# tyui592/Real_Time_Helmet_Detection

Measured on AMD Instinct MI355X. Metric: train imgs/sec, higher is better.
Workload: dtype bf16; 1 GPU; model=hourglass-1-ch128, global_batch=16, imsize=512, parallelism=dp1, engine=hip, fp8=False, hipgraph=True

## Files before the change

### real_time_helmet_detection_amd/ops/csrc/bindings.cpp

```cpp
#include <torch/extension.h>

namespace rthd {
torch::Tensor add_act_fwd(torch::Tensor a, torch::Tensor b, int64_t act);
torch::Tensor add_act_bwd(torch::Tensor dy, torch::Tensor y, int64_t act);

std::vector<torch::Tensor> pool2x2_fwd(torch::Tensor x, bool is_max,
                                       bool need_arg);
torch::Tensor pool2x2_bwd(torch::Tensor dy, torch::Tensor arg, bool is_max,
                          int64_t H, int64_t W);
std::vector<torch::Tensor> maxpool_same_fwd(torch::Tensor x, int64_t k,
                                            bool need_arg);
torch::Tensor maxpool_same_bwd(torch::Tensor dy, torch::Tensor arg,
                               int64_t k);

torch::Tensor upsample2x_add_fwd(torch::Tensor x,
                                 c10::optional<torch::Tensor> skip);
torch::Tensor upsample2x_bwd(torch::Tensor dy);

std::vector<torch::Tensor> centernet_loss_fwd(
    torch::Tensor phm, torch::Tensor poff, torch::Tensor psize,
    torch::Tensor ghm, torch::Tensor goff, torch::Tensor gsize,
    torch::Tensor mask, double alpha, double beta);
std::vector<torch::Tensor> centernet_loss_bwd(
    torch::Tensor phm, torch::Tensor poff, torch::Tensor psize,
    torch::Tensor ghm, torch::Tensor goff, torch::Tensor gsize,
    torch::Tensor mask, torch::Tensor sums, torch::Tensor gout,
    double alpha, double beta);
std::vector<torch::Tensor> centernet_loss_fused_fwd(
    torch::Tensor out, torch::Tensor ghm, torch::Tensor goff,
    torch::Tensor gsize, torch::Tensor mask, double alpha, double beta,
    bool sig_os);
torch::Tensor centernet_loss_fused_bwd(
    torch::Tensor out, torch::Tensor ghm, torch::Tensor goff,
    torch::Tensor gsize, torch::Tensor mask, torch::Tensor sums,
    torch::Tensor glosses, double alpha, double beta, bool sig_os);

std::vector<torch::Tensor> decode_fwd(torch::Tensor hm, torch::Tensor off,
                                      torch::Tensor wh, int64_t scale_factor,
                                      int64_t topk, int64_t pool_size,
                                      bool normalized);
torch::Tensor nms_fwd(torch::Tensor boxes, torch::Tensor scores,
                      double iou_threshold);
std::vector<torch::Tensor> nms_batched(torch::Tensor boxes,
                                       torch::Tensor scores,
                                       double iou_threshold,
                                       double conf_th);
std::vector<torch::Tensor> soft_nms_fwd(torch::Tensor boxes,
                                        torch::Tensor scores, double sigma,
                                        double score_th);
std::vector<torch::Tensor> soft_nms_batched(torch::Tensor boxes,
                                            torch::Tensor scores,
                                            double sigma, double score_th,
                                            double conf_th);

torch::Tensor pack_weights(torch::Tensor w, bool swap, bool to_bf16);
std::vector<torch::Tensor> pack_weights_pair(torch::Tensor w,
                                             bool to_bf16_fwd,
                                             bool to_bf16_dgrad);
torch::Tensor pack_weights_fp8(torch::Tensor w);
torch::Tensor conv_fwd_fp8r(torch::Tensor x, torch::Tensor wpk,
                            torch::Tensor scale, torch::Tensor shift,
                            c10::optional<torch::Tensor> skip,
                            int64_t KH, int64_t KW, int64_t stride,
                            int64_t pad, int64_t Cout, int64_t act,
                            bool out_fp8);
torch::Tensor conv_fwd(torch::Tensor x, torch::Tensor wpk,
                       torch::Tensor scale, torch::Tensor shift,
                       c10::optional<torch::Tensor> skip,
                       int64_t KH, int64_t KW, int64_t stride, int64_t pad,
                       int64_t Cout, int64_t act);
torch::Tensor conv_fwd_small(torch::Tensor x, torch::Tensor wpk,
                             torch::Tensor scale, torch::Tensor shift,
                             c10::optional<torch::Tensor> skip,
                             int64_t KH, int64_t KW, int64_t stride,
                             int64_t pad, int64_t Cout, int64_t act,
                             int64_t splitk);
torch::Tensor conv_fwd_k64(torch::Tensor x, torch::Tensor wpk,
                           torch::Tensor scale, torch::Tensor shift,
                           c10::optional<torch::Tensor> skip,
                           int64_t KH, int64_t KW, int64_t stride,
                           int64_t pad, int64_t Cout, int64_t act);
torch::Tensor stem_im2col(torch::Tensor x, int64_t KS, int64_t stride,
                          int64_t pad);
torch::Tensor wgrad(torch::Tensor x, torch::Tensor dy, int64_t KH,
                    int64_t KW, int64_t stride, int64_t pad);
torch::Tensor wgrad_bf16_fast(torch::Tensor x, torch::Tensor dy, int64_t KH,
                              int64_t KW, int64_t stride, int64_t pad);

std::vector<torch::Tensor> conv_fwd_stats(
    torch::Tensor x, torch::Tensor wpk, torch::Tensor scale,
    torch::Tensor shift, int64_t KH, int64_t KW, int64_t stride,
    int64_t pad, int64_t Cout, int64_t act);
std::vector<torch::Tensor> bn_stats_from_parts(
    torch::Tensor p1, torch::Tensor p2,
    c10::optional<torch::Tensor> running_mean,
    c10::optional<torch::Tensor> running_var,
    double momentum, double eps, int64_t M);
std::vector<torch::Tensor> bn_stats(torch::Tensor x,
                                    c10::optional<torch::Tensor> running_mean,
                                    c10::optional<torch::Tensor> running_var,
                                    double momentum, double eps);
torch::Tensor bn_act_fwd(torch::Tensor x, torch::Tensor mean,
                         torch::Tensor rstd, torch::Tensor gamma,
                         torch::Tensor beta, int64_t act,
                         c10::optional<torch::Tensor> skip);
std::vector<torch::Tensor> bn_act_bwd(torch::Tensor dy, torch::Tensor x,
                                      torch::Tensor mean, torch::Tensor rstd,
                                      torch::Tensor gamma, torch::Tensor beta,
                                      int64_t act,
                                      c10::optional<torch::Tensor> skip);
torch::Tensor col_sum(torch::Tensor x);

std::vector<torch::Tensor> encode_targets(torch::Tensor boxes,
                                          torch::Tensor labels, int64_t H,
                                          int64_t W, int64_t scale_factor,
                                          int64_t num_cls, bool normalized);
torch::Tensor normalize_u8(torch::Tensor img_u8, torch::Tensor table);
int64_t encode_chunk();
torch::Tensor augment_u8(torch::Tensor img_u8, torch::Tensor sizes,
                         torch::Tensor coef, int64_t T,
                         c10::optional<torch::Tensor> table);
}

PYBIND11_MODULE(TORCH_EXTENSION_NAME, m) {
  m.def("add_act_fwd", &rthd::add_act_fwd);
  m.def("add_act_bwd", &rthd::add_act_bwd);
  m.def("pool2x2_fwd", &rthd::pool2x2_fwd);
  m.def("pool2x2_bwd", &rthd::pool2x2_bwd);
  m.def("maxpool_same_fwd", &rthd::maxpool_same_fwd);
  m.def("maxpool_same_bwd", &rthd::maxpool_same_bwd);
  m.def("upsample2x_add_fwd", &rthd::upsample2x_add_fwd);
  m.def("upsample2x_bwd", &rthd::upsample2x_bwd);
  m.def("centernet_loss_fwd", &rthd::centernet_loss_fwd);
  m.def("centernet_loss_bwd", &rthd::centernet_loss_bwd);
  m.def("centernet_loss_fused_fwd", &rthd::centernet_loss_fused_fwd);
  m.def("centernet_loss_fused_bwd", &rthd::centernet_loss_fused_bwd);
  m.def("decode_fwd", &rthd::decode_fwd);
  m.def("nms_fwd", &rthd::nms_fwd);
  m.def("nms_batched", &rthd::nms_batched);
  m.def("soft_nms", &rthd::soft_nms_fwd);
  m.def("soft_nms_batched", &rthd::soft_nms_batched);
  m.def("pack_weights",&rthd::pack_weights);
  m.def("pack_weights_pair", &rthd::pack_weights_pair);
  m.def("pack_weights_fp8", &rthd::pack_weights_fp8);
  m.def("conv_fwd_fp8r", &rthd::conv_fwd_fp8r);
  m.def("conv_fwd", &rthd::conv_fwd);
  m.def("conv_fwd_small", &rthd::conv_fwd_small);
  m.def("conv_fwd_k64", &rthd::conv_fwd_k64);
  m.def("stem_im2col", &rthd::stem_im2col);
  m.def("wgrad", &rthd::wgrad);
  m.def("wgrad_bf16_fast", &rthd::wgrad_bf16_fast);
  m.def("conv_fwd_stats", &rthd::conv_fwd_stats);
  m.def("bn_stats_from_parts", &rthd::bn_stats_from_parts,
        py::arg("p1"), py::arg("p2"), py::arg("running_mean") = py::none(),
        py::arg("running_var") = py::none(), py::arg("momentum") = 0.1,
        py::arg("eps") = 1e-5, py::arg("m") = 1);
  m.def("bn_stats", &rthd::bn_stats);
  m.def("bn_act_fwd", &rthd::bn_act_fwd, py::arg("x"), py::arg("mean"), py::arg("rstd"), py::arg("gamma"), py::arg("beta"), py::arg("act"), py::arg("skip") = py::none());
  m.def("bn_act_bwd", &rthd::bn_act_bwd, py::arg("dy"), py::arg("x"), py::arg("mean"), py::arg("rstd"), py::arg("gamma"), py::arg("beta"), py::arg("act"), py::arg("skip") = py::none());
  m.def("col_sum", &rthd::col_sum);
  m.def("encode_targets", &rthd::encode_targets);
  m.def("normalize_u8", &rthd::normalize_u8);
  m.def("encode_chunk", &rthd::encode_chunk);
  m.def("augment_u8", &rthd::augment_u8, py::arg("img_u8"), py::arg("sizes"),
        py::arg("coef"), py::arg("T"), py::arg("table") = py::none());
}

namespace rthd {

static torch::Tensor maxpool2x2_op(torch::Tensor x) {
  return pool2x2_fwd(std::move(x), true, false)[0];
}
static torch::Tensor avgpool2x2_op(torch::Tensor x) {
  return pool2x2_fwd(std::move(x), false, false)[0];
}
static torch::Tensor maxpool_same_op(torch::Tensor x, int64_t k) {
  return maxpool_same_fwd(std::move(x), k, false)[0];
}
static std::tuple<torch::Tensor, torch::Tensor> nms_batched_op(
    torch::Tensor boxes, torch::Tensor scores, double iou, double conf) {
  auto v = nms_batched(std::move(boxes), std::move(scores), iou, conf);
  return {v[0], v[1]};
}
static std::tuple<torch::Tensor, torch::Tensor> soft_nms_op(
    torch::Tensor boxes, torch::Tensor scores, double sigma,
    double score_th) {
  auto v = soft_nms_fwd(std::move(boxes), std::move(scores), sigma, score_th);
  return {v[0], v[1]};
}
static std::tuple<torch::Tensor, torch::Tensor, torch::Tensor>
soft_nms_batched_op(torch::Tensor boxes, torch::Tensor scores, double sigma,
                    double score_th, double conf) {
  auto v = soft_nms_batched(std::move(boxes), std::move(scores), sigma,
                            score_th, conf);
  return {v[0], v[1], v[2]};
}
static std::tuple<torch::Tensor, torch::Tensor, torch::Tensor> decode_op(
    torch::Tensor hm, torch::Tensor off, torch::Tensor wh,
    int64_t scale_factor, int64_t topk, int64_t pool_size, bool normalized) {
  auto v = decode_fwd(std::move(hm), std::move(off), std::move(wh),
                      scale_factor, topk, pool_size, normalized);
  return {v[0], v[1], v[2]};
}

}

TORCH_LIBRARY(rthd, m) {
  m.def("conv_fwd(Tensor x, Tensor wpk, Tensor scale, Tensor shift, "
        "Tensor? skip, int kh, int kw, int stride, int pad, int cout, "
        "int act) -> Tensor");
  m.def("conv_fwd_fp8r(Tensor x, Tensor wpk, Tensor scale, Tensor shift, "
        "Tensor? skip, int kh, int kw, int stride, int pad, int cout, "
        "int act, bool out_fp8) -> Tensor");
  m.def("add_act_fwd(Tensor a, Tensor b, int act) -> Tensor");
  m.def("maxpool2x2(Tensor x) -> Tensor");
  m.def("avgpool2x2(Tensor x) -> Tensor");
  m.def("maxpool_same(Tensor x, int k) -> Tensor");
  m.def("upsample2x_add(Tensor x, Tensor? skip) -> Tensor");
  m.def("nms(Tensor boxes, Tensor scores, float iou) -> Tensor");
  m.def("nms_batched(Tensor boxes, Tensor scores, float iou, float conf) "
        "-> (Tensor, Tensor)");
  m.def("soft_nms(Tensor boxes, Tensor scores, float sigma, "
        "float score_th) -> (Tensor, Tensor)");
  m.def("soft_nms_batched(Tensor boxes, Tensor scores, float sigma, "
        "float score_th, float conf) -> (Tensor, Tensor, Tensor)");
  m.def("decode(Tensor hm, Tensor off, Tensor wh, int scale_factor, "
        "int topk, int pool_size, bool normalized) "
        "-> (Tensor, Tensor, Tensor)");
  m.def("stem_im2col(Tensor x, int ks, int stride, int pad) -> Tensor");
}

TORCH_LIBRARY_IMPL(rthd, CUDA, m) {
  m.impl("conv_fwd", rthd::conv_fwd);
  m.impl("conv_fwd_fp8r", rthd::conv_fwd_fp8r);
  m.impl("add_act_fwd", rthd::add_act_fwd);
  m.impl("maxpool2x2", rthd::maxpool2x2_op);
  m.impl("avgpool2x2", rthd::avgpool2x2_op);
  m.impl("maxpool_same", rthd::maxpool_same_op);
  m.impl("upsample2x_add", rthd::upsample2x_add_fwd);
  m.impl("nms", rthd::nms_fwd);
  m.impl("nms_batched", rthd::nms_batched_op);
  m.impl("soft_nms", rthd::soft_nms_op);
  m.impl("soft_nms_batched", rthd::soft_nms_batched_op);
  m.impl("decode", rthd::decode_op);
  m.impl("stem_im2col", rthd::stem_im2col);
}
```

### real_time_helmet_detection_amd/ops/csrc/wgrad_fast.hip

```cpp
#include <torch/extension.h>
#include <ATen/cuda/CUDAContext.h>
#include "common.h"

namespace rthd {

using bf16x8 = __attribute__((ext_vector_type(8))) short;
using f32x4 = __attribute__((ext_vector_type(4))) float;

DEV_INLINE int wg_off(int row, int px8) {
  return row * 272 + ((px8 ^ ((row >> 3) & 7)) << 4);
}

struct WgradGeo2 {
  int B, H, W, Cin, Ho, Wo, Cout;
  int KH, KW, stride, pad;
  int M;
  int chunk_len;
  int ci_tiles, co_tiles, nchunks;
};

#define WGRAD_NUM_XCD 8

template <bool ALIGNED, bool SAME>
__global__ __launch_bounds__(256)
void wgrad_bf16_kernel(const bf16* __restrict__ x,
                       const bf16* __restrict__ dy,
                       float* __restrict__ dw, WgradGeo2 g) {
  const int t = blockIdx.z % (g.KH * g.KW);
  const int chunk = blockIdx.z / (g.KH * g.KW);
  const int ci0 = blockIdx.x * 64;
  const int co0 = blockIdx.y * 64;
  const int dyt = t / g.KW - g.pad;
  const int dxt = t % g.KW - g.pad;
  const int dtoff = dyt * g.W + dxt;

  const int tid = threadIdx.x;
  const int lane = tid & 63;
  const int wid = tid >> 6;
  const int wr = wid >> 1, wc = wid & 1;

  __shared__ __attribute__((aligned(16))) char smem[2 * 64 * 272];
  bf16* Xl = reinterpret_cast<bf16*>(smem);
  bf16* Yl = reinterpret_cast<bf16*>(smem + 64 * 272);

  f32x4 acc[2][2] = {};

  const int px_start = chunk * g.chunk_len;
  const int px_end = min(px_start + g.chunk_len, g.M);

  const bool stage_x = tid < 128;
  const int s_ci = (tid & 7) * 8;
  const int s_px = ((tid >> 3) & 15) * 8;

  const int HoWo = g.Ho * g.Wo;
  int mb = px_start + s_px;
  int bb = mb / HoWo;
  int rr = mb - bb * HoWo;
  int oy = rr / g.Wo;
  int ox = rr - oy * g.Wo;

  ushort r[8][8];

#define RTHD_WG_LOADX(p0_)                                                   \
  {                                                                          \
    int bj = bb, oyj = oy, oxj = ox;                                         \
    const int cbase = ci0 + s_ci;                                            \
    _Pragma("unroll") for (int j = 0; j < 8; ++j) {                          \
      const int m = (p0_) + s_px + j;                                        \
      uint4 v;                                                               \
      const int iy = oyj * g.stride + dyt;                                   \
      const int ix = oxj * g.stride + dxt;                                   \
      const bool val = m < px_end && iy >= 0 && iy < g.H && ix >= 0 &&       \
                       ix < g.W && cbase < g.Cin;                            \
      if (ALIGNED) {                                                         \
                        \
        const int64_t off = !val ? 0                                         \
            : SAME ? (int64_t)(m + dtoff) * g.Cin + cbase                    \
            : (((int64_t)bj * g.H + iy) * g.W + ix) * g.Cin + cbase;         \
        v = *reinterpret_cast<const uint4*>(x + off);                        \
        if (!val) v = uint4{0, 0, 0, 0};                                     \
      } else {                                                               \
        v = uint4{0, 0, 0, 0};                                               \
        if (val) {                                                           \
          const ushort* src = reinterpret_cast<const ushort*>(               \
              x + (((int64_t)bj * g.H + iy) * g.W + ix) * g.Cin + cbase);    \
          ushort tmp[8] = {};                                                \
          for (int e = 0; cbase + e < g.Cin; ++e) tmp[e] = src[e];           \
          v = *reinterpret_cast<const uint4*>(tmp);                          \
        }                                                                    \
      }                                                                      \
      *reinterpret_cast<uint4*>(r[j]) = v;                                   \
      if (++oxj >= g.Wo) {                                                   \
        oxj = 0;                                                             \
        if (++oyj >= g.Ho) { oyj = 0; ++bj; }                                \
      }                                                                      \
    }                                                                        \
  }

#define RTHD_WG_LOADY(p0_)                                                   \
  {                                                                          \
    const int cbase = co0 + s_ci;                                            \
    _Pragma("unroll") for (int j = 0; j < 8; ++j) {                          \
      const int m = (p0_) + s_px + j;                                        \
      uint4 v;                                                               \
      const bool val = m < px_end && cbase < g.Cout;                         \
      if (ALIGNED) {                                                         \
        const int64_t off = val ? (int64_t)m * g.Cout + cbase : 0;           \
        v = *reinterpret_cast<const uint4*>(dy + off);                       \
        if (!val) v = uint4{0, 0, 0, 0};                                     \
      } else {                                                               \
        v = uint4{0, 0, 0, 0};                                               \
        if (val) {                                                           \
          const ushort* src = reinterpret_cast<const ushort*>(               \
              dy + (int64_t)m * g.Cout + cbase);                             \
          ushort tmp[8] = {};                                                \
          for (int e = 0; cbase + e < g.Cout; ++e) tmp[e] = src[e];          \
          v = *reinterpret_cast<const uint4*>(tmp);                          \
        }                                                                    \
      }                                                                      \
      *reinterpret_cast<uint4*>(r[j]) = v;                                   \
    }                                                                        \
  }

  if (stage_x) RTHD_WG_LOADX(px_start) else RTHD_WG_LOADY(px_start)

  for (int p0 = px_start; p0 < px_end; p0 += 128) {
    __syncthreads();
    {
      bf16* half = stage_x ? Xl : Yl;
#pragma unroll
      for (int e = 0; e < 8; ++e) {
        ushort o[8];
#pragma unroll
        for (int j = 0; j < 8; ++j) o[j] = r[j][e];
        *reinterpret_cast<uint4*>(
            reinterpret_cast<char*>(half) +
            wg_off(s_ci + e, s_px >> 3)) = *reinterpret_cast<uint4*>(o);
      }
    }
    if (stage_x) {
      ox += 128;
      while (ox >= g.Wo) {
        ox -= g.Wo;
        if (++oy >= g.Ho) { oy = 0; ++bb; }
      }
    }
    __syncthreads();
    if (p0 + 128 < px_end) {
      if (stage_x) RTHD_WG_LOADX(p0 + 128) else RTHD_WG_LOADY(p0 + 128)
    }

    asm volatile("s_setprio 1");
#pragma unroll
    for (int ks = 0; ks < 4; ++ks) {
      const int k8 = (lane >> 4) + ks * 4;
      bf16x8 xa[2], yb[2];
#pragma unroll
      for (int i = 0; i < 2; ++i) {
        const int arow = wr * 32 + i * 16 + (lane & 15);
        xa[i] = *reinterpret_cast<const bf16x8*>(
            reinterpret_cast<char*>(Xl) + wg_off(arow, k8));
        const int brow = wc * 32 + i * 16 + (lane & 15);
        yb[i] = *reinterpret_cast<const bf16x8*>(
            reinterpret_cast<char*>(Yl) + wg_off(brow, k8));
      }
#pragma unroll
      for (int mi = 0; mi < 2; ++mi)
#pragma unroll
        for (int ni = 0; ni < 2; ++ni)
          acc[mi][ni] = __builtin_amdgcn_mfma_f32_16x16x32_bf16(
              xa[mi], yb[ni], acc[mi][ni], 0, 0, 0);
    }
    asm volatile("s_setprio 0");
  }

#undef RTHD_WG_LOADX
#undef RTHD_WG_LOADY

  const int ty = t / g.KW, tx = t % g.KW;
  float* dwc = dw + (int64_t)chunk * g.Cout * g.Cin * g.KH * g.KW;
#pragma unroll
  for (int mi = 0; mi < 2; ++mi) {
#pragma unroll
    for (int r2 = 0; r2 < 4; ++r2) {
      const int ci = ci0 + wr * 32 + mi * 16 + (lane >> 4) * 4 + r2;
      if (ci >= g.Cin) continue;
#pragma unroll
      for (int ni = 0; ni < 2; ++ni) {
        const int co = co0 + wc * 32 + ni * 16 + (lane & 15);
        if (co >= g.Cout) continue;
        dwc[(((int64_t)co * g.KH + ty) * g.KW + tx) * g.Cin + ci] =
            acc[mi][ni][r2];
      }
    }
  }
}

__global__ void wgrad_reduce_kernel(const float* __restrict__ part,
                                    float* __restrict__ out,
                                    int K, int64_t N) {
  const int64_t n4 = N >> 2;
  for (int64_t i = blockIdx.x * (int64_t)blockDim.x + threadIdx.x;
       i < n4; i += (int64_t)gridDim.x * blockDim.x) {
    float4 a = {0.f, 0.f, 0.f, 0.f};
    int k = 0;
    for (; k + 3 < K; k += 4) {
      float4 v[4];
#pragma unroll
      for (int u = 0; u < 4; ++u)
        v[u] = *reinterpret_cast<const float4*>(
            &part[(int64_t)(k + u) * N + i * 4]);
#pragma unroll
      for (int u = 0; u < 4; ++u) {
        a.x += v[u].x; a.y += v[u].y; a.z += v[u].z; a.w += v[u].w;
      }
    }
    for (; k < K; ++k) {
      const float4 v =
          *reinterpret_cast<const float4*>(&part[(int64_t)k * N + i * 4]);
      a.x += v.x; a.y += v.y; a.z += v.z; a.w += v.w;
    }
    *reinterpret_cast<float4*>(&out[i * 4]) = a;
  }
  for (int64_t i = n4 * 4 + blockIdx.x * (int64_t)blockDim.x + threadIdx.x;
       i < N; i += (int64_t)gridDim.x * blockDim.x) {
    float a = 0.f;
    for (int k = 0; k < K; ++k) a += part[(int64_t)k * N + i];
    out[i] = a;
  }
}

torch::Tensor wgrad_bf16_fast(torch::Tensor x, torch::Tensor dy, int64_t KH,
                              int64_t KW, int64_t stride, int64_t pad) {
  auto xc = x.contiguous(at::MemoryFormat::ChannelsLast);
  auto dyc = dy.to(at::kBFloat16).contiguous(at::MemoryFormat::ChannelsLast);
  WgradGeo2 g;
  g.B = xc.size(0);
  g.Cin = xc.size(1);
  g.H = xc.size(2);
  g.W = xc.size(3);
  g.Cout = dyc.size(1);
  g.Ho = dyc.size(2);
  g.Wo = dyc.size(3);
  g.KH = KH; g.KW = KW; g.stride = stride; g.pad = pad;
  g.M = g.B * g.Ho * g.Wo;

  const int ci_tiles = (int)cdiv(g.Cin, 64);
  const int co_tiles = (int)cdiv(g.Cout, 64);
  const int taps = (int)(KH * KW);
  int nchunks = std::max(1, 1024 / (ci_tiles * co_tiles * taps));
  int chunk_len = (int)cdiv(g.M, nchunks);
  chunk_len = (int)cdiv(chunk_len, 128) * 128;
  if (taps == 1 && g.M >= 4096) chunk_len = std::max(chunk_len, 2048);
  if (const char* e = getenv("RTHD_WGRAD_CHUNK")) {
    const int v = atoi(e);
    if (v >= 128) chunk_len = (int)cdiv(v, 128) * 128;
  }
  nchunks = (int)cdiv(g.M, chunk_len);
  g.chunk_len = chunk_len;
  g.ci_tiles = ci_tiles;
  g.co_tiles = co_tiles;
  g.nchunks = nchunks;

  const int64_t N = (int64_t)g.Cout * g.Cin * KH * KW;
  auto dwp = torch::empty({(int64_t)nchunks * N},
                          xc.options().dtype(at::kFloat));
  auto dw = torch::empty({g.Cout, g.Cin, KH, KW},
                         xc.options().dtype(at::kFloat).memory_format(
                             at::MemoryFormat::ChannelsLast));

  dim3 grid(ci_tiles, co_tiles, taps * nchunks);
  auto s = at::cuda::getCurrentCUDAStream();
  const bool aligned = (g.Cin % 8 == 0) && (g.Cout % 8 == 0);
  const bool same = stride == 1 && g.Ho == g.H && g.Wo == g.W;
  auto* px = reinterpret_cast<const bf16*>(xc.data_ptr());
  auto* pdy = reinterpret_cast<const bf16*>(dyc.data_ptr());
#define RTHD_WG_LAUNCH(A_, S_)                                           \
  hipLaunchKernelGGL((wgrad_bf16_kernel<A_, S_>), grid, dim3(256), 0, s, \
      px, pdy, dwp.data_ptr<float>(), g)
  if (aligned && same) RTHD_WG_LAUNCH(true, true);
  else if (aligned)    RTHD_WG_LAUNCH(true, false);
  else if (same)       RTHD_WG_LAUNCH(false, true);
  else                 RTHD_WG_LAUNCH(false, false);
#undef RTHD_WG_LAUNCH
  const int rblocks = (int)std::min<int64_t>(2048, cdiv(N, 4 * 256) + 1);
  hipLaunchKernelGGL(wgrad_reduce_kernel, dim3(rblocks), dim3(256), 0, s,
      dwp.data_ptr<float>(), dw.data_ptr<float>(), nchunks, N);
  HIP_CHECK_LAST();
  return dw;
}

}
```

Before: 1110 imgs/sec.

## Add transposed-LDS-read wgrad kernel with triple-buffered async loads as default path

```diff
diff --git a/real_time_helmet_detection_amd/ops/csrc/bindings.cpp b/real_time_helmet_detection_amd/ops/csrc/bindings.cpp
--- a/real_time_helmet_detection_amd/ops/csrc/bindings.cpp
+++ b/real_time_helmet_detection_amd/ops/csrc/bindings.cpp
@@ -85,7 +85,12 @@
 torch::Tensor wgrad(torch::Tensor x, torch::Tensor dy, int64_t KH,
                     int64_t KW, int64_t stride, int64_t pad);
 torch::Tensor wgrad_bf16_fast(torch::Tensor x, torch::Tensor dy, int64_t KH,
-                              int64_t KW, int64_t stride, int64_t pad);
+                              int64_t KW, int64_t stride, int64_t pad,
+                              const std::string& variant);
+torch::Tensor lds_tr16_selftest();
+std::string wgrad_bf16_choice(int64_t Cin, int64_t Cout, int64_t M);
+int64_t wgrad_bf16_chunk_len(int64_t Cin, int64_t Cout, int64_t taps,
+                             int64_t M);
 
 std::vector<torch::Tensor> conv_fwd_stats(
     torch::Tensor x, torch::Tensor wpk, torch::Tensor scale,
@@ -149,7 +154,12 @@
   m.def("conv_fwd_k64", &rthd::conv_fwd_k64);
   m.def("stem_im2col", &rthd::stem_im2col);
   m.def("wgrad", &rthd::wgrad);
-  m.def("wgrad_bf16_fast", &rthd::wgrad_bf16_fast);
+  m.def("wgrad_bf16_fast", &rthd::wgrad_bf16_fast,
+        py::arg("x"), py::arg("dy"), py::arg("kh"), py::arg("kw"),
+        py::arg("stride"), py::arg("pad"), py::arg("variant") = "");
+  m.def("lds_tr16_selftest", &rthd::lds_tr16_selftest);
+  m.def("wgrad_bf16_choice", &rthd::wgrad_bf16_choice);
+  m.def("wgrad_bf16_chunk_len", &rthd::wgrad_bf16_chunk_len);
   m.def("conv_fwd_stats", &rthd::conv_fwd_stats);
   m.def("bn_stats_from_parts", &rthd::bn_stats_from_parts,
         py::arg("p1"), py::arg("p2"), py::arg("running_mean") = py::none(),
diff --git a/real_time_helmet_detection_amd/ops/csrc/wgrad_fast.hip b/real_time_helmet_detection_amd/ops/csrc/wgrad_fast.hip
--- a/real_time_helmet_detection_amd/ops/csrc/wgrad_fast.hip
+++ b/real_time_helmet_detection_amd/ops/csrc/wgrad_fast.hip
@@ -1,8 +1,14 @@
 #include <torch/extension.h>
 #include <ATen/cuda/CUDAContext.h>
 #include "common.h"
+#include "wgrad_tr_geo.h"
 
 namespace rthd {
+
+const bf16* zero_page_bf16(const torch::Tensor& like);
+void wgrad_tr_launch(const WtrGeo& g, int nchunks, const bf16* x,
+                     const bf16* dy, const bf16* zpage, float* dwp,
+                     hipStream_t s);
 
 using bf16x8 = __attribute__((ext_vector_type(8))) short;
 using f32x4 = __attribute__((ext_vector_type(4))) float;
@@ -230,8 +236,27 @@
   }
 }
 
+static bool wgrad_default_is_tr(int Cin, int Cout, int M) {
+  constexpr int kTrMinPx = 4096;
+  const char* e = getenv("RTHD_WGRAD_REGT");
+  const bool force_regt = e && atoi(e) != 0;
+  return Cin % 8 == 0 && Cout % 8 == 0 && !force_regt && M > kTrMinPx;
+}
+
+std::string wgrad_bf16_choice(int64_t Cin, int64_t Cout, int64_t M) {
+  return wgrad_default_is_tr((int)Cin, (int)Cout, (int)M) ? "tr" : "regt";
+}
+
+int64_t wgrad_bf16_chunk_len(int64_t Cin, int64_t Cout, int64_t taps,
+                             int64_t M) {
+  int forced = 0;
+  if (const char* e = getenv("RTHD_WGRAD_CHUNK")) forced = atoi(e);
+  return wtr_chunk_len((int)M, (int)Cin, (int)Cout, (int)taps, forced);
+}
+
 torch::Tensor wgrad_bf16_fast(torch::Tensor x, torch::Tensor dy, int64_t KH,
-                              int64_t KW, int64_t stride, int64_t pad) {
+                              int64_t KW, int64_t stride, int64_t pad,
+                              const std::string& variant) {
   auto xc = x.contiguous(at::MemoryFormat::ChannelsLast);
   auto dyc = dy.to(at::kBFloat16).contiguous(at::MemoryFormat::ChannelsLast);
   WgradGeo2 g;
@@ -248,15 +273,8 @@
   const int ci_tiles = (int)cdiv(g.Cin, 64);
   const int co_tiles = (int)cdiv(g.Cout, 64);
   const int taps = (int)(KH * KW);
-  int nchunks = std::max(1, 1024 / (ci_tiles * co_tiles * taps));
-  int chunk_len = (int)cdiv(g.M, nchunks);
-  chunk_len = (int)cdiv(chunk_len, 128) * 128;
-  if (taps == 1 && g.M >= 4096) chunk_len = std::max(chunk_len, 2048);
-  if (const char* e = getenv("RTHD_WGRAD_CHUNK")) {
-    const int v = atoi(e);
-    if (v >= 128) chunk_len = (int)cdiv(v, 128) * 128;
-  }
-  nchunks = (int)cdiv(g.M, chunk_len);
+  const int chunk_len = (int)wgrad_bf16_chunk_len(g.Cin, g.Cout, taps, g.M);
+  const int nchunks = (int)cdiv(g.M, chunk_len);
   g.chunk_len = chunk_len;
   g.ci_tiles = ci_tiles;
   g.co_tiles = co_tiles;
@@ -272,13 +290,34 @@
   dim3 grid(ci_tiles, co_tiles, taps * nchunks);
   auto s = at::cuda::getCurrentCUDAStream();
   const bool aligned = (g.Cin % 8 == 0) && (g.Cout % 8 == 0);
+
+  bool use_tr = false;
+  if (variant == "tr") {
+    TORCH_CHECK(aligned, "wgrad_bf16_fast: variant 'tr' needs Cin % 8 == 0 "
+                "and Cout % 8 == 0");
+    use_tr = true;
+  } else if (variant.empty()) {
+    use_tr = wgrad_default_is_tr(g.Cin, g.Cout, g.M);
+  } else {
+    TORCH_CHECK(variant == "regt", "wgrad_bf16_fast: unknown variant '",
+                variant, "'");
+  }
   const bool same = stride == 1 && g.Ho == g.H && g.Wo == g.W;
   auto* px = reinterpret_cast<const bf16*>(xc.data_ptr());
   auto* pdy = reinterpret_cast<const bf16*>(dyc.data_ptr());
 #define RTHD_WG_LAUNCH(A_, S_)                                           \
   hipLaunchKernelGGL((wgrad_bf16_kernel<A_, S_>), grid, dim3(256), 0, s, \
       px, pdy, dwp.data_ptr<float>(), g)
-  if (aligned && same) RTHD_WG_LAUNCH(true, true);
+  if (use_tr) {
+    WtrGeo tg;
+    tg.B = g.B; tg.H = g.H; tg.W = g.W; tg.Cin = g.Cin;
+    tg.Ho = g.Ho; tg.Wo = g.Wo; tg.Cout = g.Cout;
+    tg.KH = g.KH; tg.KW = g.KW; tg.stride = g.stride; tg.pad = g.pad;
+    tg.M = g.M; tg.chunk_len = g.chunk_len;
+    wgrad_tr_launch(tg, nchunks, px, pdy, zero_page_bf16(xc),
+                    dwp.data_ptr<float>(), s);
+  }
+  else if (aligned && same) RTHD_WG_LAUNCH(true, true);
   else if (aligned)    RTHD_WG_LAUNCH(true, false);
   else if (same)       RTHD_WG_LAUNCH(false, true);
   else                 RTHD_WG_LAUNCH(false, false);
diff --git a/real_time_helmet_detection_amd/ops/csrc/wgrad_tr.hip b/real_time_helmet_detection_amd/ops/csrc/wgrad_tr.hip
--- /dev/null
+++ b/real_time_helmet_detection_amd/ops/csrc/wgrad_tr.hip
@@ -0,0 +1,276 @@
+#include <mutex>
+
+#include "conv_common.h"
+#include "wgrad_tr_geo.h"
+
+namespace rthd {
+
+namespace {
+
+using i16x4 = __attribute__((ext_vector_type(4))) short;
+typedef __attribute__((address_space(3))) i16x4 lds_i16x4;
+
+typedef __attribute__((address_space(3))) char lds_char;
+
+constexpr int WTR_NBUF = 3;
+constexpr int WTR_NUM_XCD = 8;
+
+template <int OFF>
+DEV_INLINE i16x4 tr_read(uint32_t addr) {
+  i16x4 v;
+  asm volatile("ds_read_b64_tr_b16 %0, %1 offset:%2"
+               : "=v"(v) : "v"(addr), "n"(OFF) : "memory");
+  return v;
+}
+
+DEV_INLINE bf16x8 tr_read_frag(const char* p0, const char* p1) {
+  const i16x4 lo = __builtin_amdgcn_ds_read_tr16_b64_v4i16((lds_i16x4*)p0);
+  const i16x4 hi = __builtin_amdgcn_ds_read_tr16_b64_v4i16((lds_i16x4*)p1);
+  return __builtin_shufflevector(lo, hi, 0, 1, 2, 3, 4, 5, 6, 7);
+}
+
+__global__ __launch_bounds__(64)
+void lds_tr16_selftest_kernel(short* __restrict__ out) {
+  __shared__ __attribute__((aligned(16))) short img[32 * 64];
+  const int lane = threadIdx.x;
+  for (int i = lane; i < 32 * 64; i += 64) img[i] = (short)i;
+  __syncthreads();
+  const int g = lane >> 4, q = (lane >> 2) & 3, p = lane & 3;
+  const char* base = reinterpret_cast<const char*>(img);
+#pragma unroll
+  for (int cb = 0; cb < 4; ++cb) {
+    const int a0 = ((8 * g + q) * 64 + 16 * cb + 4 * p) * 2;
+    const bf16x8 v = tr_read_frag(base + a0, base + a0 + 4 * 64 * 2);
+    *reinterpret_cast<bf16x8*>(out + (cb * 64 + lane) * 8) = v;
+  }
+}
+
+template <int BM, int BN>
+__global__ __launch_bounds__(256)
+void wgrad_tr_kernel(const bf16* __restrict__ x, const bf16* __restrict__ dy,
+                     const bf16* __restrict__ zpage, float* __restrict__ dw,
+                     WtrGeo g, int xcd_remap) {
+  constexpr int MI = BM / 32, NI = BN / 32;
+  constexpr int XB = WTR_KB * BM * 2;
+  constexpr int YB = WTR_KB * BN * 2;
+  constexpr int STAGE = XB + YB;
+  constexpr int NX = XB / 4096;
+  constexpr int NY = YB / 4096;
+  constexpr int KS = WTR_KB / 32;
+  constexpr int RD1 = 2 * (MI + NI);
+  static_assert(KS == 2, "the fragment reads below are written for KS = 2");
+  extern __shared__ __attribute__((aligned(16))) char smem[];
+
+  const int taps = g.KH * g.KW;
+  const int ci_t = (g.Cin + BM - 1) / BM, co_t = (g.Cout + BN - 1) / BN;
+  int cell = blockIdx.x;
+  if (xcd_remap) {
+    const int G = gridDim.x, k = cell % WTR_NUM_XCD, j = cell / WTR_NUM_XCD;
+    cell = k * (G / WTR_NUM_XCD) + min(k, G % WTR_NUM_XCD) + j;
+  }
+  const int z = cell / (ci_t * co_t);
+  const int t = z % taps;
+  const int chunk = z / taps;
+  const int ci0 = (cell % ci_t) * BM;
+  const int co0 = (cell / ci_t % co_t) * BN;
+  const int dyt = t / g.KW - g.pad;
+  const int dxt = t % g.KW - g.pad;
+
+  const int tid = threadIdx.x;
+  const int lane = tid & 63;
+  const int wid = tid >> 6;
+  const int wr = wid >> 1, wc = wid & 1;
+
+  const int px_start = chunk * g.chunk_len;
+  const int px_end = min(px_start + g.chunk_len, g.M);
+  const int nsteps = (px_end - px_start + WTR_KB - 1) / WTR_KB;
+
+  WtrPix pix[NX];
+  int xrow[NX], xch[NX], yrow[NY], ych[NY];
+#pragma unroll
+  for (int i = 0; i < NX; ++i) {
+    int c;
+    wtr_stage_slot(i * 4 + wid, lane, BM, &xrow[i], &c);
+    xch[i] = ci0 + c * 8;
+    wtr_pix_init(px_start + xrow[i], g.Ho, g.Wo, &pix[i]);
+  }
+#pragma unroll
+  for (int i = 0; i < NY; ++i) {
+    int c;
+    wtr_stage_slot(i * 4 + wid, lane, BN, &yrow[i], &c);
+    ych[i] = co0 + c * 8;
+  }
+  const int adv_b = WTR_KB / (g.Ho * g.Wo);
+  const int adv_q = WTR_KB % (g.Ho * g.Wo) / g.Wo, adv_r = WTR_KB % g.Wo;
+
+  auto issue_step = [&](int step, int buf) {
+    char* base = smem + buf * STAGE;
+    const int p0 = px_start + step * WTR_KB;
+#pragma unroll
+    for (int i = 0; i < NX; ++i) {
+      const int64_t off = wtr_x_src(g, pix[i], p0 + xrow[i], px_end, dyt,
+                                    dxt, xch[i]);
+      const bf16* src = off < 0 ? zpage : x + off;
+      __builtin_amdgcn_global_load_lds((glb_void*)src,
+          (lds_void*)(base + wtr_stage_byte(i * 4 + wid, lane)), 16, 0, 0);
+      wtr_pix_advance(&pix[i], adv_b, adv_q, adv_r, g.Ho, g.Wo);
+    }
+#pragma unroll
+    for (int i = 0; i < NY; ++i) {
+      const int64_t off = wtr_dy_src(g, p0 + yrow[i], px_end, ych[i]);
+      const bf16* src = off < 0 ? zpage : dy + off;
+      __builtin_amdgcn_global_load_lds((glb_void*)src,
+          (lds_void*)(base + XB + wtr_stage_byte(i * 4 + wid, lane)),
+          16, 0, 0);
+    }
+  };
+
+  const uint32_t lds0 = (uint32_t)(uintptr_t)(lds_char*)smem;
+  uint32_t aoff[MI][2], boff[NI][2];
+#pragma unroll
+  for (int h = 0; h < 2; ++h) {
+#pragma unroll
+    for (int mi = 0; mi < MI; ++mi)
+      aoff[mi][h] = lds0 + wtr_tr_addr(wr * MI + mi, 0, h, lane, BM);
+#pragma unroll
+    for (int ni = 0; ni < NI; ++ni)
+      boff[ni][h] = lds0 + XB + wtr_tr_addr(wc * NI + ni, 0, h, lane, BN);
+  }
+
+  f32x4 acc[MI][NI] = {};
+
+  issue_step(0, 0);
+  if (nsteps > 1) issue_step(1, 1);
+  int rbuf = 0;
+
+  for (int step = 0; step < nsteps; ++step) {
+    if (step + 1 < nsteps)
+      asm volatile("s_waitcnt vmcnt(%0)" ::"n"(NX + NY) : "memory");
+    else
+      asm volatile("s_waitcnt vmcnt(0)" ::: "memory");
+    __builtin_amdgcn_s_barrier();
+
+    const uint32_t boffs = (uint32_t)(rbuf * STAGE);
+    i16x4 xlo[KS][MI], xhi[KS][MI], ylo[KS][NI], yhi[KS][NI];
+#pragma unroll
+    for (int mi = 0; mi < MI; ++mi) {
+      xlo[0][mi] = tr_read<0>(aoff[mi][0] + boffs);
+      xhi[0][mi] = tr_read<0>(aoff[mi][1] + boffs);
+    }
+#pragma unroll
+    for (int ni = 0; ni < NI; ++ni) {
+      ylo[0][ni] = tr_read<0>(boff[ni][0] + boffs);
+      yhi[0][ni] = tr_read<0>(boff[ni][1] + boffs);
+    }
+#pragma unroll
+    for (int mi = 0; mi < MI; ++mi) {
+      xlo[1][mi] = tr_read<32 * BM * 2>(aoff[mi][0] + boffs);
+      xhi[1][mi] = tr_read<32 * BM * 2>(aoff[mi][1] + boffs);
+    }
+#pragma unroll
+    for (int ni = 0; ni < NI; ++ni) {
+      ylo[1][ni] = tr_read<32 * BN * 2>(boff[ni][0] + boffs);
+      yhi[1][ni] = tr_read<32 * BN * 2>(boff[ni][1] + boffs);
+    }
+
+    const int wbuf = rbuf == 0 ? 2 : rbuf - 1;
+    if (step + 2 < nsteps) issue_step(step + 2, wbuf);
+    rbuf = rbuf == 2 ? 0 : rbuf + 1;
+
+    __builtin_amdgcn_sched_barrier(0);
+    __builtin_amdgcn_s_setprio(1);
+#pragma unroll
+    for (int ks = 0; ks < KS; ++ks) {
+      if (ks == 0)
+        asm volatile("s_waitcnt lgkmcnt(%0)" ::"n"(RD1 < 15 ? RD1 : 15));
+      else
+        asm volatile("s_waitcnt lgkmcnt(0)");
+#pragma unroll
+      for (int mi = 0; mi < MI; ++mi)
+        asm volatile("" : "+v"(xlo[ks][mi]), "+v"(xhi[ks][mi]));
+#pragma unroll
+      for (int ni = 0; ni < NI; ++ni)
+        asm volatile("" : "+v"(ylo[ks][ni]), "+v"(yhi[ks][ni]));
+      __builtin_amdgcn_sched_barrier(0);
+      bf16x8 xa[MI], yb[NI];
+#pragma unroll
+      for (int mi = 0; mi < MI; ++mi)
+        xa[mi] = __builtin_shufflevector(xlo[ks][mi], xhi[ks][mi], 0, 1, 2,
+                                         3, 4, 5, 6, 7);
+#pragma unroll
+      for (int ni = 0; ni < NI; ++ni)
+        yb[ni] = __builtin_shufflevector(ylo[ks][ni], yhi[ks][ni], 0, 1, 2,
+                                         3, 4, 5, 6, 7);
+#pragma unroll
+      for (int mi = 0; mi < MI; ++mi)
+#pragma unroll
+        for (int ni = 0; ni < NI; ++ni)
+          acc[mi][ni] = __builtin_amdgcn_mfma_f32_16x16x32_bf16(
+              xa[mi], yb[ni], acc[mi][ni], 0, 0, 0);
+      __builtin_amdgcn_sched_barrier(0);
+    }
+    __builtin_amdgcn_s_setprio(0);
+    __builtin_amdgcn_sched_barrier(0);
+  }
+
+  const int ty = t / g.KW, tx = t % g.KW;
+  float* dwc = dw + (int64_t)chunk * g.Cout * g.Cin * taps;
+#pragma unroll
+  for (int mi = 0; mi < MI; ++mi) {
+#pragma unroll
+    for (int r = 0; r < 4; ++r) {
+      const int ci = ci0 + (wr * MI + mi) * 16 + (lane >> 4) * 4 + r;
+      if (ci >= g.Cin) continue;
+#pragma unroll
+      for (int ni = 0; ni < NI; ++ni) {
+        const int co = co0 + (wc * NI + ni) * 16 + (lane & 15);
+        if (co >= g.Cout) continue;
+        dwc[(((int64_t)co * g.KH + ty) * g.KW + tx) * g.Cin + ci] =
+            acc[mi][ni][r];
+      }
+    }
+  }
+}
+
+}
+
+constexpr int WTR_BM = 64, WTR_BN = 128;
+
+void wgrad_tr_launch(const WtrGeo& g, int nchunks, const bf16* x,
+                     const bf16* dy, const bf16* zpage, float* dwp,
+                     hipStream_t s) {
+  const dim3 grid((unsigned)(cdiv(g.Cin, WTR_BM) * cdiv(g.Cout, WTR_BN) *
+                             g.KH * g.KW * nchunks));
+  const int remap = g.M >= 65536;
+  const size_t lds = (size_t)WTR_NBUF * WTR_KB * (WTR_BM + WTR_BN) * 2;
+  {
+    static std::mutex mu;
+    static uint64_t done = 0;
+    int dev = 0;
+    TORCH_CHECK(hipGetDevice(&dev) == hipSuccess && dev < 64,
+                "wgrad_tr: bad device");
+    std::lock_guard<std::mutex> lk(mu);
+    if (!((done >> dev) & 1)) {
+      const hipError_t e = hipFuncSetAttribute(
+          reinterpret_cast<const void*>(&wgrad_tr_kernel<WTR_BM, WTR_BN>),
+          hipFuncAttributeMaxDynamicSharedMemorySize, (int)lds);
+      TORCH_CHECK(e == hipSuccess, "wgrad_tr: cannot opt in to ", lds,
+                  " B of LDS: ", hipGetErrorString(e));
+      done |= (uint64_t)1 << dev;
+    }
+  }
+  hipLaunchKernelGGL((wgrad_tr_kernel<WTR_BM, WTR_BN>), grid, dim3(256), lds,
+                     s, x, dy, zpage, dwp, g, remap);
+}
+
+torch::Tensor lds_tr16_selftest() {
+  auto out = torch::empty({4, 64, 8}, torch::dtype(torch::kInt16)
+                                          .device(torch::kCUDA));
+  hipLaunchKernelGGL(lds_tr16_selftest_kernel, dim3(1), dim3(64), 0,
+                     at::cuda::getCurrentCUDAStream(),
+                     out.data_ptr<int16_t>());
+  HIP_CHECK_LAST();
+  return out;
+}
+
+}
diff --git a/real_time_helmet_detection_amd/ops/csrc/wgrad_tr_geo.h b/real_time_helmet_detection_amd/ops/csrc/wgrad_tr_geo.h
--- /dev/null
+++ b/real_time_helmet_detection_amd/ops/csrc/wgrad_tr_geo.h
@@ -0,0 +1,93 @@
+#pragma once
+
+#include <cstdint>
+
+#if defined(__HIPCC__)
+#define WTR_HD __host__ __device__ inline
+#else
+#define WTR_HD inline
+#endif
+
+namespace rthd {
+
+constexpr int WTR_KB = 64;
+
+struct WtrGeo {
+  int B, H, W, Cin, Ho, Wo, Cout;
+  int KH, KW, stride, pad;
+  int M;
+  int chunk_len;
+};
+
+WTR_HD int wtr_chunk_len(int M, int Cin, int Cout, int taps, int forced) {
+  const int tiles = ((Cin + 63) / 64) * ((Cout + 63) / 64) * taps;
+  const int nchunks = 1024 / tiles > 1 ? 1024 / tiles : 1;
+  int len = ((M + nchunks - 1) / nchunks + 127) / 128 * 128;
+  if (taps == 1 && M >= 4096 && len < 2048) len = 2048;
+  if (forced >= 128) len = (forced + 127) / 128 * 128;
+  return len;
+}
+
+WTR_HD int wtr_swz(int row, int CH) {
+  return CH == 128 ? (((row & 3) << 2) | ((row >> 2) & 3))
+                   : ((((row >> 1) & 1) << 2) | (((row >> 3) & 1) << 1));
+}
+
+WTR_HD int wtr_lds_off(int row, int chunk, int CH) {
+  return row * (CH * 2) + ((chunk ^ wtr_swz(row, CH)) << 4);
+}
+
+WTR_HD int wtr_stage_byte(int f, int lane) { return f * 1024 + lane * 16; }
+
+WTR_HD void wtr_stage_slot(int f, int lane, int CH, int* row, int* chunk) {
+  const int byte = wtr_stage_byte(f, lane);
+  const int r = byte / (CH * 2);
+  const int pc = (byte % (CH * 2)) >> 4;
+  *row = r;
+  *chunk = pc ^ wtr_swz(r, CH);
+}
+
+WTR_HD int wtr_tr_addr(int frag, int ks, int h, int lane, int CH) {
+  const int g = lane >> 4, q = (lane >> 2) & 3, p = lane & 3;
+  const int row = 32 * ks + 8 * g + 4 * h + q;
+  return wtr_lds_off(row, 2 * frag + (p >> 1), CH) + 8 * (p & 1);
+}
+
+struct WtrPix { int b, oy, ox; };
+
+WTR_HD void wtr_pix_init(int m, int Ho, int Wo, WtrPix* p) {
+  p->b = m / (Ho * Wo);
+  const int r = m - p->b * (Ho * Wo);
+  p->oy = r / Wo;
+  p->ox = r - p->oy * Wo;
+}
+
+WTR_HD void wtr_pix_advance(WtrPix* p, int db, int dq, int dr, int Ho,
+                            int Wo) {
+  int ox = p->ox + dr;
+  const int cx = ox >= Wo;
+  ox -= cx ? Wo : 0;
+  int oy = p->oy + dq + cx;
+  const int cy = oy >= Ho;
+  oy -= cy ? Ho : 0;
+  p->ox = ox;
+  p->oy = oy;
+  p->b += db + cy;
+}
+
+WTR_HD int64_t wtr_x_src(const WtrGeo& g, const WtrPix& p, int m, int px_end,
+                         int dyt, int dxt, int c) {
+  const int iy = p.oy * g.stride + dyt;
+  const int ix = p.ox * g.stride + dxt;
+  const bool ok = (m < px_end) & (iy >= 0) & (iy < g.H) & (ix >= 0) &
+                  (ix < g.W) & (c < g.Cin);
+  const int64_t off = (int64_t)((p.b * g.H + iy) * g.W + ix) * g.Cin + c;
+  return ok ? off : -1;
+}
+
+WTR_HD int64_t wtr_dy_src(const WtrGeo& g, int m, int px_end, int c) {
+  const bool ok = (m < px_end) & (c < g.Cout);
+  return ok ? (int64_t)m * g.Cout + c : -1;
+}
+
+}
```

Result: faster. 1181 imgs/sec (median of 6 runs) (+6.4%).
